# spacemeshos/go-spacemesh

Hardware: AMD Instinct MI355X
Metric: post_labels_per_sec (higher is better)
Workload: dtype u32; 1 GPU; init-mainnet-scryptN8192-4units-256GiB-sink; step_labels=2097152, scrypt_n=8192, num_units=4, labels_per_unit=4294967296, parallelism=index-range shards x1, RCCL nonce min-reduce, vrf_nonce_found=True

## Files before the change

### go-spacemesh_amd/csrc/engine.cpp

```cpp
#include "../../include/spacemesh_post.h"

#include <hip/hip_runtime.h>

#include <fcntl.h>
#include <sys/stat.h>
#include <sys/types.h>
#include <unistd.h>

#include <algorithm>
#include <array>
#include <atomic>
#include <thread>
#include <chrono>
#include <cerrno>
#include <cstdio>
#include <cstdlib>
#include <cstring>
#include <functional>
#include <map>
#include <mutex>
#include <string>
#include <vector>

#include "crypto_host.h"
#include "kernel_args.h"
#include "post_common.h"

namespace {

thread_local std::string g_last_error;

void set_error(const std::string &e) { g_last_error = e; }

int hip_fail(const char *what, hipError_t err) {
  set_error(std::string(what) + ": " + hipGetErrorString(err));
  return err == hipErrorOutOfMemory ? POST_ERR_OOM : POST_ERR;
}

#define HIP_TRY(expr)                                                          \
  do {                                                                         \
    hipError_t _e = (expr);                                                    \
    if (_e != hipSuccess) return hip_fail(#expr, _e);                          \
  } while (0)

int require_gpu(uint32_t provider_id) {
  int count = 0;
  hipError_t e = hipGetDeviceCount(&count);
  if (e != hipSuccess || count == 0) {
    set_error("no HIP device available (the HIP engine has no CPU fallback)");
    return POST_ERR_NO_GPU;
  }
  if (provider_id >= (uint32_t)count) {
    set_error("provider id out of range");
    return POST_ERR_INVALID_ARGS;
  }
  e = hipSetDevice((int)provider_id);
  if (e != hipSuccess) return hip_fail("hipSetDevice", e);
  return POST_OK;
}

void load_commitment_words(const uint8_t c[32], uint32_t w[8]) {
  std::memcpy(w, c, 32);
}

void difficulty_to_be_words(const uint8_t d[32], uint32_t w[8]) {
  for (int i = 0; i < 8; i++)
    w[i] = ((uint32_t)d[4 * i] << 24) | ((uint32_t)d[4 * i + 1] << 16) |
           ((uint32_t)d[4 * i + 2] << 8) | d[4 * i + 3];
}

constexpr uint32_t THREADS = 256;
constexpr uint32_t CAND_CAP = 1 << 16;

uint32_t pick_gap_shift(uint32_t scrypt_n) {
  const char *env = getenv("POST_GAP_SHIFT");
  if (env) {
    uint32_t g = (uint32_t)atoi(env);
    while ((scrypt_n >> g) == 0) g--;
    return g;
  }
  return 0;
}

uint64_t prove_chunk_labels() {
  const uint64_t dflt = 1ull << 24;
  const char *env = getenv("POST_PROVE_CHUNK_LABELS");
  if (!env) return dflt;
  const long long v = strtoll(env, nullptr, 10);
  if (v <= 0 || (uint64_t)v >= dflt) return dflt;
  return v < 256 ? 256 : (uint64_t)v;
}

struct VerifyWorkspace {
  std::mutex mu;
  uint32_t *d_scratch = nullptr;
  size_t scratch_cap = 0;
  uint64_t *d_idx = nullptr;
  uint32_t *d_cid = nullptr;
  uint8_t *d_out = nullptr;
  uint32_t *d_xbuf = nullptr;
  size_t tasks_cap = 0;
  uint32_t *d_cm = nullptr;
  size_t cm_cap = 0;
  uint32_t *d_vrk = nullptr;
  uint8_t *d_half = nullptr;
  uint64_t *d_vdiff = nullptr;
  size_t proofs_cap = 0;
  uint8_t *d_pass = nullptr;
};
std::mutex g_vws_mu;
std::map<int, VerifyWorkspace *> g_vws;

VerifyWorkspace *get_verify_ws(int dev) {
  std::lock_guard<std::mutex> lk(g_vws_mu);
  auto it = g_vws.find(dev);
  if (it != g_vws.end()) return it->second;
  auto *w = new VerifyWorkspace();
  g_vws[dev] = w;
  return w;
}

int ws_reserve_proofs(VerifyWorkspace *w, size_t proofs) {
  if (proofs > w->proofs_cap) {
    size_t cap = std::max<size_t>(proofs, 1024);
    if (w->d_vrk) (void)hipFree(w->d_vrk);
    if (w->d_half) (void)hipFree(w->d_half);
    if (w->d_vdiff) (void)hipFree(w->d_vdiff);
    w->d_vrk = nullptr; w->d_half = nullptr; w->d_vdiff = nullptr;
    w->proofs_cap = 0;
    HIP_TRY(hipMalloc(&w->d_vrk, cap * 44 * 4));
    HIP_TRY(hipMalloc(&w->d_half, cap));
    HIP_TRY(hipMalloc(&w->d_vdiff, cap * 8));
    w->proofs_cap = cap;
  }
  return POST_OK;
}

int ws_reserve(VerifyWorkspace *w, size_t scratch_bytes, size_t tasks,
               size_t cm_words) {
  if (scratch_bytes > w->scratch_cap) {
    if (w->d_scratch) (void)hipFree(w->d_scratch);
    w->d_scratch = nullptr;
    w->scratch_cap = 0;
    HIP_TRY(hipMalloc(&w->d_scratch, scratch_bytes));
    w->scratch_cap = scratch_bytes;
  }
  if (tasks > w->tasks_cap) {
    size_t cap = std::max<size_t>(tasks, 4096);
    if (w->d_idx) (void)hipFree(w->d_idx);
    if (w->d_cid) (void)hipFree(w->d_cid);
    if (w->d_out) (void)hipFree(w->d_out);
    if (w->d_xbuf) (void)hipFree(w->d_xbuf);
    if (w->d_pass) (void)hipFree(w->d_pass);
    w->d_idx = nullptr; w->d_cid = nullptr; w->d_out = nullptr;
    w->d_xbuf = nullptr; w->d_pass = nullptr;
    w->tasks_cap = 0;
    HIP_TRY(hipMalloc(&w->d_idx, cap * 8));
    HIP_TRY(hipMalloc(&w->d_cid, cap * 4));
    HIP_TRY(hipMalloc(&w->d_out, cap * 32));
    HIP_TRY(hipMalloc(&w->d_xbuf, cap * 128));
    HIP_TRY(hipMalloc(&w->d_pass, cap));
    w->tasks_cap = cap;
  }
  if (cm_words > w->cm_cap) {
    size_t cap = std::max<size_t>(cm_words, 1024);
    if (w->d_cm) (void)hipFree(w->d_cm);
    w->d_cm = nullptr;
    w->cm_cap = 0;
    HIP_TRY(hipMalloc(&w->d_cm, cap * 4));
    w->cm_cap = cap;
  }
  return POST_OK;
}

struct DeviceTables {
  uint32_t *d_te = nullptr;
  uint8_t *d_sbox = nullptr;
};
std::mutex g_tables_mu;
std::map<int, DeviceTables> g_tables;

int get_aes_tables(int dev, DeviceTables &out) {
  std::lock_guard<std::mutex> lk(g_tables_mu);
  auto it = g_tables.find(dev);
  if (it != g_tables.end()) {
    out = it->second;
    return POST_OK;
  }
  static uint32_t te[1024];
  static uint8_t sbox[256];
  poste::aes128_tables(te, sbox);
  DeviceTables t;
  HIP_TRY(hipMalloc(&t.d_te, sizeof(te)));
  HIP_TRY(hipMalloc(&t.d_sbox, sizeof(sbox)));
  HIP_TRY(hipMemcpy(t.d_te, te, sizeof(te), hipMemcpyHostToDevice));
  HIP_TRY(hipMemcpy(t.d_sbox, sbox, sizeof(sbox), hipMemcpyHostToDevice));
  g_tables[dev] = t;
  out = t;
  return POST_OK;
}

}

extern "C" {

const char *post_last_error(void) { return g_last_error.c_str(); }

const char *post_engine_version(void) {
  return "spacemesh-post-hip 0.2 (gfx950)";
}


int post_providers(PostProvider *providers, uint32_t cap, uint32_t *count) {
  int n = 0;
  hipError_t e = hipGetDeviceCount(&n);
  if (e != hipSuccess) n = 0;
  *count = (uint32_t)n;
  for (uint32_t i = 0; i < (uint32_t)n && i < cap; i++) {
    hipDeviceProp_t prop;
    if (hipGetDeviceProperties(&prop, (int)i) != hipSuccess) continue;
    providers[i].id = i;
    std::snprintf(providers[i].model, sizeof(providers[i].model), "%s",
                  prop.name);
    providers[i].device_type = 0;
    providers[i].memory_bytes = prop.totalGlobalMem;
    providers[i].performance = 0;
  }
  return POST_OK;
}


struct PostInitSession {
  PostInitConfig cfg;
  std::string data_dir;
  uint64_t range_start = 0, range_end = 0;
  std::atomic<uint64_t> written{0};
  std::atomic<bool> cancel{false};
  uint8_t commitment[32];

  std::mutex nonce_mu;
  bool nonce_found = false;
  uint64_t nonce_idx = 0;
  uint8_t nonce_label[32];

  uint64_t lanes = 0;
  uint64_t batch_seq = 0;
  uint32_t gap_shift = 0;
  uint64_t batch = 0;
  uint32_t *d_scratch = nullptr;
  uint8_t *d_out = nullptr;
  uint8_t *d_all = nullptr;
  bool keep_all = false;
  PostVrfCandidate *d_cand = nullptr;
  unsigned int *d_cand_count = nullptr;
  uint32_t *d_xbuf = nullptr;
  uint8_t *h_batch = nullptr;
  hipStream_t stream = nullptr;
  hipEvent_t ev0 = nullptr, ev1 = nullptr;
  double last_kernel_ms = 0;

  int split_streams = 0;
  uint32_t cand_cap = 0;
  uint8_t *d_out1 = nullptr;
  PostVrfCandidate *d_cand1 = nullptr;
  unsigned int *d_cand_count1 = nullptr;
  uint8_t *h_batch1 = nullptr;
  PostVrfCandidate *h_cand[2] = {nullptr, nullptr};
  unsigned int *h_cand_count = nullptr;
  hipStream_t stream_b = nullptr, copy_stream = nullptr;
  hipEvent_t ev_fill[4] = {nullptr, nullptr, nullptr, nullptr};
  hipEvent_t ev_tail[2][2] = {{nullptr, nullptr}, {nullptr, nullptr}};
  hipEvent_t ev_end[2] = {nullptr, nullptr}, ev_done[2] = {nullptr, nullptr};

  ~PostInitSession() {
    if (stream) (void)hipStreamSynchronize(stream);
    if (stream_b) (void)hipStreamSynchronize(stream_b);
    if (copy_stream) (void)hipStreamSynchronize(copy_stream);
    for (int i = 0; i < 4; i++)
      if (ev_fill[i]) (void)hipEventDestroy(ev_fill[i]);
    for (int i = 0; i < 2; i++) {
      for (int k = 0; k < 2; k++)
        if (ev_tail[i][k]) (void)hipEventDestroy(ev_tail[i][k]);
      if (ev_end[i]) (void)hipEventDestroy(ev_end[i]);
      if (ev_done[i]) (void)hipEventDestroy(ev_done[i]);
      if (h_cand[i]) (void)hipHostFree(h_cand[i]);
    }
    if (stream_b) (void)hipStreamDestroy(stream_b);
    if (copy_stream) (void)hipStreamDestroy(copy_stream);
    if (d_out1) (void)hipFree(d_out1);
    if (d_cand1) (void)hipFree(d_cand1);
    if (d_cand_count1) (void)hipFree(d_cand_count1);
    if (h_batch1) (void)hipHostFree(h_batch1);
    if (h_cand_count) (void)hipHostFree(h_cand_count);
    if (ev0) (void)hipEventDestroy(ev0);
    if (ev1) (void)hipEventDestroy(ev1);
    if (stream) (void)hipStreamDestroy(stream);
    if (d_scratch) (void)hipFree(d_scratch);
    if (d_out) (void)hipFree(d_out);
    if (d_all) (void)hipFree(d_all);
    if (d_cand) (void)hipFree(d_cand);
    if (d_cand_count) (void)hipFree(d_cand_count);
    if (d_xbuf) (void)hipFree(d_xbuf);
    if (h_batch) (void)hipHostFree(h_batch);
  }
};

static uint64_t existing_labels(const std::string &dir, uint64_t per_file,
                                uint64_t range_start, uint64_t range_total) {
  uint64_t done = 0;
  for (uint64_t pos = range_start; pos < range_start + range_total;) {
    uint64_t file_i = pos / per_file;
    uint64_t in_file = pos % per_file;
    uint64_t file_cap = std::min(per_file - in_file,
                                 range_start + range_total - pos);
    char path[4096];
    std::snprintf(path, sizeof path, "%s/postdata_%llu.bin", dir.c_str(),
                  (unsigned long long)file_i);
    FILE *f = std::fopen(path, "rb");
    if (!f) break;
    std::fseek(f, 0, SEEK_END);
    long sz = std::ftell(f);
    std::fclose(f);
    uint64_t labels_here = (uint64_t)(sz < 0 ? 0 : sz) / POST_LABEL_SIZE;
    if (in_file > labels_here) break;
    uint64_t usable = std::min(labels_here - in_file, file_cap);
    done += usable;
    pos += usable;
    if (usable < file_cap) break;
  }
  return done;
}

static int check_existing_metadata(PostInitSession *s);
static int write_metadata(PostInitSession *s);

int post_init_new(const PostInitConfig *cfg, PostInitSession **out) {
  if (!cfg || !out) {
    set_error("null args");
    return POST_ERR_INVALID_ARGS;
  }
  if (cfg->scrypt_n < 2 || (cfg->scrypt_n & (cfg->scrypt_n - 1))) {
    set_error("scrypt N must be a power of two >= 2");
    return POST_ERR_INVALID_ARGS;
  }
  int rc = require_gpu(cfg->provider_id);
  if (rc != POST_OK) return rc;

  struct Guard {
    PostInitSession *p;
    ~Guard() { delete p; }
  };
  auto *s = new PostInitSession();
  Guard guard{s};
  s->cfg = *cfg;
  if (cfg->data_dir) {
    s->data_dir = cfg->data_dir;
    std::string path;
    for (size_t i = 0; i <= s->data_dir.size(); i++) {
      if (i == s->data_dir.size() || s->data_dir[i] == '/') {
        path = s->data_dir.substr(0, i);
        if (!path.empty()) (void)::mkdir(path.c_str(), 0755);
      }
    }
    struct stat st;
    if (stat(s->data_dir.c_str(), &st) != 0 || !S_ISDIR(st.st_mode)) {
      set_error("cannot create data dir " + s->data_dir);
      return POST_ERR_IO;
    }
  }
  uint64_t total = (uint64_t)cfg->num_units * cfg->labels_per_unit;
  s->range_start = cfg->index_start;
  s->range_end = cfg->index_end ? cfg->index_end : total;
  if (s->range_end > total || s->range_start >= s->range_end) {
    set_error("bad index range");
    return POST_ERR_INVALID_ARGS;
  }
  poste::commitment(cfg->node_id, cfg->commitment_atx_id, s->commitment);

  s->gap_shift = pick_gap_shift(cfg->scrypt_n);
  size_t free_b = 0, total_b = 0;
  HIP_TRY(hipMemGetInfo(&free_b, &total_b));
  uint64_t budget = cfg->scratch_bytes
                        ? cfg->scratch_bytes
                        : (uint64_t)((double)free_b * 0.80);
  uint64_t per_lane = ((uint64_t)cfg->scrypt_n >> s->gap_shift) * 128;
  uint64_t lanes = budget / per_lane;
  uint64_t range = s->range_end - s->range_start;
  lanes = std::min<uint64_t>(lanes, std::max<uint64_t>(range, 64));
  lanes = std::min<uint64_t>(lanes,
                             poste_label_resident_slots(s->gap_shift));
  lanes = (lanes / 128) * 128;
  if (lanes == 0) lanes = 128;
  if (lanes == 0) {
    set_error("not enough device memory for one scratch lane block");
    return POST_ERR_OOM;
  }
  s->lanes = lanes;
  s->batch = std::min<uint64_t>(range, lanes * 4);

  HIP_TRY(hipMalloc(&s->d_scratch, (size_t)lanes * per_lane));
  uint64_t keep_bytes = range * POST_LABEL_SIZE;
  s->keep_all = s->data_dir.empty() && keep_bytes <= (8ull << 30);
  if (s->keep_all) {
    HIP_TRY(hipMalloc(&s->d_all, (size_t)keep_bytes));
  }
  HIP_TRY(hipMalloc(&s->d_out, (size_t)s->batch * POST_LABEL_SIZE));
  s->cand_cap =
      (uint32_t)std::max<uint64_t>(CAND_CAP, s->batch / 64 + 16);
  HIP_TRY(hipMalloc(&s->d_cand, sizeof(PostVrfCandidate) * s->cand_cap));
  HIP_TRY(hipMalloc(&s->d_xbuf,
                    (size_t)std::max<uint64_t>(s->batch, lanes) * 128));
  HIP_TRY(hipMalloc(&s->d_cand_count, sizeof(unsigned int)));
  HIP_TRY(hipHostMalloc(&s->h_batch, (size_t)s->batch * POST_LABEL_SIZE));
  HIP_TRY(hipStreamCreate(&s->stream));

  {
    const char *mx = getenv("POST_ROMIX_MIX");
    const bool lean = poste_label_romix_lean_ok(cfg->scrypt_n, s->gap_shift,
                                                lanes) != 0;
    if (!lean || (mx && std::strcmp(mx, "0") == 0))
      s->split_streams = 0;
    else if (mx && std::strcmp(mx, "seq") == 0)
      s->split_streams = 1;
    else
      s->split_streams = lanes >= 128 ? 2 : 0;
  }
  if (s->split_streams) {
    if (!s->keep_all)
      HIP_TRY(hipMalloc(&s->d_out1, (size_t)s->batch * POST_LABEL_SIZE));
    HIP_TRY(hipMalloc(&s->d_cand1, sizeof(PostVrfCandidate) * s->cand_cap));
    HIP_TRY(hipMalloc(&s->d_cand_count1, sizeof(unsigned int)));
    HIP_TRY(hipHostMalloc(&s->h_batch1, (size_t)s->batch * POST_LABEL_SIZE));
    HIP_TRY(hipHostMalloc(&s->h_cand_count, 2 * sizeof(unsigned int)));
    for (int i = 0; i < 2; i++) {
      HIP_TRY(hipHostMalloc(&s->h_cand[i],
                            sizeof(PostVrfCandidate) * s->cand_cap));
      HIP_TRY(hipEventCreate(&s->ev_end[i]));
      HIP_TRY(hipEventCreateWithFlags(&s->ev_done[i], hipEventDisableTiming));
      for (int k = 0; k < 2; k++)
        HIP_TRY(hipEventCreateWithFlags(&s->ev_tail[i][k],
                                        hipEventDisableTiming));
    }
    for (int i = 0; i < 4; i++)
      HIP_TRY(hipEventCreateWithFlags(&s->ev_fill[i], hipEventDisableTiming));
    if (s->split_streams == 2) HIP_TRY(hipStreamCreate(&s->stream_b));
    HIP_TRY(hipStreamCreate(&s->copy_stream));
  }

  if (!s->data_dir.empty()) {
    rc = check_existing_metadata(s);
    if (rc != POST_OK) return rc;
    rc = write_metadata(s);
    if (rc != POST_OK) return rc;
    uint64_t per_file = std::max<uint64_t>(
        1, s->cfg.max_file_size / POST_LABEL_SIZE);
    s->written = existing_labels(s->data_dir, per_file, s->range_start, range);
  }
  guard.p = nullptr;
  *out = s;
  return POST_OK;
}

uint64_t post_init_num_labels_written(const PostInitSession *s) {
  return s ? s->written.load() : 0;
}

void post_init_cancel(PostInitSession *s) {
  if (s) s->cancel = true;
}

int post_init_nonce(const PostInitSession *s, uint64_t *index,
                    uint8_t label[32]) {
  auto *m = const_cast<PostInitSession *>(s);
  std::lock_guard<std::mutex> lk(m->nonce_mu);
  if (!s->nonce_found) return POST_ERR;
  *index = s->nonce_idx;
  std::memcpy(label, s->nonce_label, 32);
  return POST_OK;
}

static int write_batch_files(PostInitSession *s, uint64_t pos, uint64_t count,
                             const uint8_t *host_labels) {
  uint64_t per_file =
      std::max<uint64_t>(1, s->cfg.max_file_size / POST_LABEL_SIZE);
  uint64_t off = 0;
  while (off < count) {
    uint64_t gpos = pos + off;
    uint64_t file_i = gpos / per_file;
    uint64_t in_file = gpos % per_file;
    uint64_t take = std::min(per_file - in_file, count - off);
    char path[4096];
    std::snprintf(path, sizeof path, "%s/postdata_%llu.bin",
                  s->data_dir.c_str(), (unsigned long long)file_i);
    FILE *f = std::fopen(path, "r+b");
    if (!f) f = std::fopen(path, "w+b");
    if (!f) {
      set_error(std::string("cannot open ") + path);
      return POST_ERR_IO;
    }
    std::fseek(f, (long)(in_file * POST_LABEL_SIZE), SEEK_SET);
    size_t wr = std::fwrite(host_labels + off * POST_LABEL_SIZE,
                            POST_LABEL_SIZE, take, f);
    std::fclose(f);
    if (wr != take) {
      set_error("short write");
      return POST_ERR_IO;
    }
    off += take;
  }
  return POST_OK;
}

static void b64(const uint8_t *in, size_t n, std::string &out) {
  static const char t[] =
      "ABCDEFGHIJKLMNOPQRSTUVWXYZabcdefghijklmnopqrstuvwxyz0123456789+/";
  for (size_t i = 0; i < n; i += 3) {
    uint32_t v = (uint32_t)in[i] << 16;
    if (i + 1 < n) v |= (uint32_t)in[i + 1] << 8;
    if (i + 2 < n) v |= in[i + 2];
    out += t[(v >> 18) & 63];
    out += t[(v >> 12) & 63];
    out += i + 1 < n ? t[(v >> 6) & 63] : '=';
    out += i + 2 < n ? t[v & 63] : '=';
  }
}

static bool b64_decode(const std::string &in, uint8_t *out, size_t want) {
  static int8_t rev[256];
  static bool init = false;
  if (!init) {
    static const char t[] =
        "ABCDEFGHIJKLMNOPQRSTUVWXYZabcdefghijklmnopqrstuvwxyz0123456789+/";
    for (int i = 0; i < 256; i++) rev[i] = -1;
    for (int i = 0; i < 64; i++) rev[(uint8_t)t[i]] = (int8_t)i;
    init = true;
  }
  size_t n = 0;
  uint32_t acc = 0;
  int bits = 0;
  for (char c : in) {
    if (c == '=') break;
    int8_t v = rev[(uint8_t)c];
    if (v < 0) return false;
    acc = (acc << 6) | (uint32_t)v;
    bits += 6;
    if (bits >= 8) {
      bits -= 8;
      if (n >= want) return false;
      out[n++] = (uint8_t)(acc >> bits);
    }
  }
  return n == want;
}

static bool md_find_string(const std::string &j, const char *key,
                           std::string &out) {
  std::string pat = std::string("\"") + key + "\": \"";
  size_t p = j.find(pat);
  if (p == std::string::npos) return false;
  p += pat.size();
  size_t e = j.find('"', p);
  if (e == std::string::npos) return false;
  out = j.substr(p, e - p);
  return true;
}

static bool md_find_u64(const std::string &j, const char *key,
                        uint64_t &out) {
  std::string pat = std::string("\"") + key + "\": ";
  size_t p = j.find(pat);
  if (p == std::string::npos) return false;
  out = strtoull(j.c_str() + p + pat.size(), nullptr, 10);
  return true;
}

static int check_existing_metadata(PostInitSession *s) {
  char path[4096];
  std::snprintf(path, sizeof path, "%s/postdata_metadata.json",
                s->data_dir.c_str());
  FILE *f = std::fopen(path, "rb");
  if (!f) return POST_OK;
  std::string j;
  char buf[4096];
  size_t rd;
  while ((rd = std::fread(buf, 1, sizeof buf, f)) > 0) j.append(buf, rd);
  std::fclose(f);
  std::string nid_b64, atx_b64, want_nid, want_atx;
  b64(s->cfg.node_id, 32, want_nid);
  b64(s->cfg.commitment_atx_id, 32, want_atx);
  uint64_t lpu = 0, n = 0;
  if (md_find_string(j, "NodeId", nid_b64) && nid_b64 != want_nid) {
    set_error("data dir belongs to a different node id (postdata_metadata"
              ".json mismatch)");
    return POST_ERR_INVALID_ARGS;
  }
  if (md_find_string(j, "CommitmentAtxId", atx_b64) &&
      atx_b64 != want_atx) {
    set_error("data dir was initialized for a different commitment ATX");
    return POST_ERR_INVALID_ARGS;
  }
  if (md_find_u64(j, "LabelsPerUnit", lpu) &&
      lpu != s->cfg.labels_per_unit) {
    set_error("data dir was initialized with a different LabelsPerUnit");
    return POST_ERR_INVALID_ARGS;
  }
  if (md_find_u64(j, "N", n) && n != s->cfg.scrypt_n) {
    set_error("data dir was initialized with different scrypt params");
    return POST_ERR_INVALID_ARGS;
  }
  uint64_t nonce_idx = 0;
  std::string nv_b64;
  if (md_find_u64(j, "Nonce", nonce_idx) &&
      md_find_string(j, "NonceValue", nv_b64)) {
    uint8_t label[32];
    if (!b64_decode(nv_b64, label, 32)) {
      set_error("postdata_metadata.json NonceValue is not 32 base64 bytes");
      return POST_ERR_INVALID_ARGS;
    }
    std::lock_guard<std::mutex> lk(s->nonce_mu);
    s->nonce_found = true;
    s->nonce_idx = nonce_idx;
    std::memcpy(s->nonce_label, label, 32);
  }
  return POST_OK;
}

static int write_metadata(PostInitSession *s) {
  std::string nid, atx, nv;
  b64(s->cfg.node_id, 32, nid);
  b64(s->cfg.commitment_atx_id, 32, atx);
  char path[4096];
  std::snprintf(path, sizeof path, "%s/postdata_metadata.json",
                s->data_dir.c_str());
  FILE *f = std::fopen(path, "w");
  if (!f) {
    set_error("cannot write metadata");
    return POST_ERR_IO;
  }
  std::fprintf(f,
               "{\n  \"NodeId\": \"%s\",\n  \"CommitmentAtxId\": \"%s\",\n"
               "  \"LabelsPerUnit\": %llu,\n  \"NumUnits\": %u,\n"
               "  \"MaxFileSize\": %llu,\n  \"Scrypt\": {\"N\": %u, \"R\": 1,"
               " \"P\": 1}",
               nid.c_str(), atx.c_str(),
               (unsigned long long)s->cfg.labels_per_unit, s->cfg.num_units,
               (unsigned long long)s->cfg.max_file_size, s->cfg.scrypt_n);
  std::lock_guard<std::mutex> lk(s->nonce_mu);
  if (s->nonce_found) {
    b64(s->nonce_label, 32, nv);
    std::fprintf(f, ",\n  \"Nonce\": %llu,\n  \"NonceValue\": \"%s\"",
                 (unsigned long long)s->nonce_idx, nv.c_str());
  }
  std::fprintf(f, "\n}\n");
  std::fclose(f);
  return POST_OK;
}

static int init_step_split(PostInitSession *s, uint64_t max_labels,
                           uint64_t *done) {
  const int ns = s->split_streams;
  const uint64_t unit = s->lanes / (uint64_t)ns;
  hipStream_t st[2] = {s->stream, s->stream_b};
  uint8_t *const d_outs[2] = {s->d_out, s->d_out1};
  uint8_t *const h_batches[2] = {s->h_batch, s->h_batch1};
  PostVrfCandidate *const d_cands[2] = {s->d_cand, s->d_cand1};
  unsigned int *const d_counts[2] = {s->d_cand_count, s->d_cand_count1};

  auto drain = [&] {
    for (int k = 0; k < ns; k++) (void)hipStreamSynchronize(st[k]);
    (void)hipStreamSynchronize(s->copy_stream);
  };
#define SPLIT_TRY(expr)                                                        \
  do {                                                                         \
    hipError_t _e = (expr);                                                    \
    if (_e != hipSuccess) {                                                    \
      drain();                                                                 \
      return hip_fail(#expr, _e);                                              \
    }                                                                          \
  } while (0)

  LabelKernelArgs args;
  std::memset(&args, 0, sizeof(args));
  load_commitment_words(s->commitment, args.commitment_le);
  args.scrypt_n = s->cfg.scrypt_n;
  args.gap_shift = s->gap_shift;
  args.scratch = s->d_scratch;
  args.scratch_lanes = s->lanes;
  args.has_difficulty = 1;
  args.cand_cap = s->cand_cap;
  RomixPhaseArgs ph;
  std::memset(&ph, 0, sizeof(ph));
  ph.scratch = s->d_scratch;
  ph.scratch_lanes = s->lanes;
  ph.slot_count = unit;
  ph.scrypt_n = s->cfg.scrypt_n;

  uint8_t cur_difficulty[32];
  std::memset(cur_difficulty, 0xff, 32);
  {
    std::lock_guard<std::mutex> lk(s->nonce_mu);
    if (s->nonce_found) std::memcpy(cur_difficulty, s->nonce_label, 32);
  }
  const char *sp_env = getenv("POST_SELFCHECK_PERIOD");
  long selfcheck_period = sp_env ? strtol(sp_env, nullptr, 10) : 1;
  if (selfcheck_period < 1) selfcheck_period = 1;

  if (!s->ev0) SPLIT_TRY(hipEventCreate(&s->ev0));
  s->last_kernel_ms = 0;

  struct Batch {
    uint64_t pos = 0, count = 0;
    uint32_t max_cand = 0;
    int set = 0;
    bool live = false;
  };
  uint64_t unit_seq = 0;
  uint64_t batch_no = 0;
  int last_set = -1;

  auto issue = [&](Batch &b) -> int {
    b.set = (int)(batch_no++ & 1);
    b.max_cand = 0;
    uint8_t *out =
        s->keep_all ? s->d_all + b.pos * POST_LABEL_SIZE : d_outs[b.set];
    args.cand = d_cands[b.set];
    args.cand_count = d_counts[b.set];
    difficulty_to_be_words(cur_difficulty, args.difficulty_be);
    SPLIT_TRY(hipMemsetAsync(d_counts[b.set], 0, sizeof(unsigned int),
                             st[unit_seq % ns]));
    bool used[2] = {false, false};
    for (uint64_t off = 0; off < b.count; off += unit) {
      const int k = (int)(unit_seq % (uint64_t)ns);
      const uint64_t c = std::min(unit, b.count - off);
      const uint32_t blocks = (uint32_t)((c + 63) / 64);
      args.start = s->range_start + b.pos + off;
      args.count = c;
      args.xbuf = s->d_xbuf + (uint64_t)k * unit * 32;
      args.out = out + off * POST_LABEL_SIZE;
      ph.xbuf = args.xbuf;
      ph.slot_base = (uint64_t)k * unit;
      ph.count = c;
      if (unit_seq == 0) SPLIT_TRY(hipEventRecord(s->ev0, st[k]));
      SPLIT_TRY(poste_launch_label_prologue(&args, blocks, st[k]));
      if (ns == 2 && unit_seq > 0)
        SPLIT_TRY(hipStreamWaitEvent(st[k], s->ev_fill[(unit_seq - 1) & 3],
                                     0));
      SPLIT_TRY(poste_launch_romix_fill(&ph, st[k]));
      if (ns == 2)
        SPLIT_TRY(hipEventRecord(s->ev_fill[unit_seq & 3], st[k]));
      SPLIT_TRY(poste_launch_romix_mix(&ph, st[k]));
      SPLIT_TRY(poste_launch_label_tail(&args, blocks, st[k]));
      b.max_cand += blocks;
      used[k] = true;
      unit_seq++;
    }
    for (int k = 0; k < ns; k++) {
      if (!used[k]) continue;
      SPLIT_TRY(hipEventRecord(s->ev_tail[b.set][k], st[k]));
      SPLIT_TRY(hipStreamWaitEvent(s->copy_stream, s->ev_tail[b.set][k], 0));
    }
    SPLIT_TRY(hipEventRecord(s->ev_end[b.set], s->copy_stream));
    SPLIT_TRY(hipMemcpyAsync(h_batches[b.set], out,
                             b.count * POST_LABEL_SIZE, hipMemcpyDeviceToHost,
                             s->copy_stream));
    SPLIT_TRY(hipMemcpyAsync(s->h_cand_count + b.set, d_counts[b.set],
                             sizeof(unsigned int), hipMemcpyDeviceToHost,
                             s->copy_stream));
    b.max_cand = std::min(b.max_cand, s->cand_cap);
    SPLIT_TRY(hipMemcpyAsync(s->h_cand[b.set], d_cands[b.set],
                             sizeof(PostVrfCandidate) * b.max_cand,
                             hipMemcpyDeviceToHost, s->copy_stream));
    SPLIT_TRY(hipEventRecord(s->ev_done[b.set], s->copy_stream));
    last_set = b.set;
    b.live = true;
    return POST_OK;
  };

  auto process = [&](Batch &b) -> int {
    b.live = false;
    const bool do_selfcheck =
        (s->batch_seq++ % (uint64_t)selfcheck_period) == 0;
    const uint64_t probe = b.count / 2;
    uint8_t ref[32];
    const int ref_rc =
        do_selfcheck
            ? poste::host_label(s->commitment, s->range_start + b.pos + probe,
                                s->cfg.scrypt_n, ref)
            : 0;
    SPLIT_TRY(hipEventSynchronize(s->ev_done[b.set]));
    const unsigned int take = std::min(s->h_cand_count[b.set], b.max_cand);
    const PostVrfCandidate *cands = s->h_cand[b.set];
    bool nonce_improved = false;
    if (take > 0) {
      std::lock_guard<std::mutex> lk(s->nonce_mu);
      for (unsigned int i = 0; i < take; i++) {
        uint8_t lab[32];
        for (int k = 0; k < 8; k++) {
          uint32_t w = cands[i].label_be[k];
          lab[4 * k] = (uint8_t)(w >> 24);
          lab[4 * k + 1] = (uint8_t)(w >> 16);
          lab[4 * k + 2] = (uint8_t)(w >> 8);
          lab[4 * k + 3] = (uint8_t)w;
        }
        int c = std::memcmp(lab, cur_difficulty, 32);
        if (!s->nonce_found || c < 0 ||
            (c == 0 && cands[i].index < s->nonce_idx)) {
          s->nonce_found = true;
          s->nonce_idx = cands[i].index;
          std::memcpy(s->nonce_label, lab, 32);
          std::memcpy(cur_difficulty, lab, 32);
          nonce_improved = true;
        }
      }
    }
    int rc = POST_OK;
    if (nonce_improved && !s->data_dir.empty()) rc = write_metadata(s);
    if (rc == POST_OK && ref_rc != 0) {
      set_error("host reference label failed");
      rc = POST_ERR;
    }
    if (rc == POST_OK && do_selfcheck &&
        std::memcmp(ref, h_batches[b.set] + probe * POST_LABEL_SIZE,
                    POST_LABEL_SIZE) != 0) {
      set_error("reference label mismatch: device labels diverge from the "
                "host reference (ErrReferenceLabelMismatch)");
      rc = POST_ERR;
    }
    if (rc == POST_OK && !s->data_dir.empty())
      rc = write_batch_files(s, s->range_start + b.pos, b.count,
                             h_batches[b.set]);
    if (rc != POST_OK) {
      drain();
      return rc;
    }
    s->written.store(b.pos + b.count);
    *done += b.count;
    return POST_OK;
  };

  const uint64_t range = s->range_end - s->range_start;
  uint64_t pos = s->written.load();
  const uint64_t target = std::min(range, pos + max_labels);
  Batch inflight[2];
  int cur = 0;
  bool cancelled = false;
  while (pos < target) {
    if (s->cancel.load()) {
      cancelled = true;
      break;
    }
    Batch &b = inflight[cur];
    b.pos = pos;
    b.count = std::min(s->batch, target - pos);
    int rc = issue(b);
    if (rc != POST_OK) return rc;
    pos += b.count;
    if (inflight[cur ^ 1].live) {
      rc = process(inflight[cur ^ 1]);
      if (rc != POST_OK) return rc;
    }
    cur ^= 1;
  }
  if (inflight[cur ^ 1].live) {
    int rc = process(inflight[cur ^ 1]);
    if (rc != POST_OK) return rc;
  }
  drain();
  if (last_set >= 0) {
    float ms = 0;
    (void)hipEventElapsedTime(&ms, s->ev0, s->ev_end[last_set]);
    s->last_kernel_ms = ms;
  }
#undef SPLIT_TRY
  return cancelled ? POST_ERR_CANCELLED : POST_OK;
}

int post_init_step(PostInitSession *s, uint64_t max_labels, uint64_t *done) {
  if (!s || !done) return POST_ERR_INVALID_ARGS;
  *done = 0;
  int rc = require_gpu(s->cfg.provider_id);
  if (rc != POST_OK) return rc;
  if (s->split_streams) return init_step_split(s, max_labels, done);

  LabelKernelArgs args;
  std::memset(&args, 0, sizeof(args));
  load_commitment_words(s->commitment, args.commitment_le);
  args.scrypt_n = s->cfg.scrypt_n;
  args.gap_shift = s->gap_shift;
  args.xbuf = s->d_xbuf;
  args.out_full = 0;
  args.scratch = s->d_scratch;
  args.scratch_lanes = s->lanes;
  args.indices = nullptr;
  args.commit_ids = nullptr;
  args.commitments = nullptr;
  args.has_difficulty = 1;
  args.cand = s->d_cand;
  args.cand_count = s->d_cand_count;
  args.cand_cap = s->cand_cap;

  uint8_t cur_difficulty[32];
  std::memset(cur_difficulty, 0xff, 32);
  {
    std::lock_guard<std::mutex> lk(s->nonce_mu);
    if (s->nonce_found) std::memcpy(cur_difficulty, s->nonce_label, 32);
  }

  const uint32_t blocks = (uint32_t)(s->lanes / 64);
  std::vector<PostVrfCandidate> cands(s->cand_cap);

  if (!s->ev0) {
    HIP_TRY(hipEventCreate(&s->ev0));
    HIP_TRY(hipEventCreate(&s->ev1));
  }
  s->last_kernel_ms = 0;

  uint64_t range = s->range_end - s->range_start;
  uint64_t pos = s->written.load();
  uint64_t target = std::min(range, pos + max_labels);
  while (pos < target) {
    if (s->cancel.load()) return POST_ERR_CANCELLED;
    uint64_t count = std::min(s->batch, target - pos);
    args.start = s->range_start + pos;
    args.count = count;
    args.out = s->keep_all ? s->d_all + pos * POST_LABEL_SIZE : s->d_out;
    difficulty_to_be_words(cur_difficulty, args.difficulty_be);
    unsigned int zero = 0;
    HIP_TRY(hipMemcpyAsync(s->d_cand_count, &zero, sizeof(zero),
                           hipMemcpyHostToDevice, s->stream));
    HIP_TRY(hipEventRecord(s->ev0, s->stream));
    HIP_TRY(poste_launch_label_kernel(&args, blocks, s->stream));
    HIP_TRY(hipEventRecord(s->ev1, s->stream));
    HIP_TRY(hipMemcpyAsync(s->h_batch, args.out, count * POST_LABEL_SIZE,
                           hipMemcpyDeviceToHost, s->stream));
    unsigned int n_cand = 0;
    HIP_TRY(hipMemcpyAsync(&n_cand, s->d_cand_count, sizeof(n_cand),
                           hipMemcpyDeviceToHost, s->stream));
    const char *sp_env = getenv("POST_SELFCHECK_PERIOD");
    long selfcheck_period = sp_env ? strtol(sp_env, nullptr, 10) : 1;
    if (selfcheck_period < 1) selfcheck_period = 1;
    const bool do_selfcheck = (s->batch_seq++ % (uint64_t)selfcheck_period)
                              == 0;
    const uint64_t probe = count / 2;
    uint8_t ref[32];
    const int ref_rc =
        do_selfcheck ? poste::host_label(s->commitment, args.start + probe,
                                         s->cfg.scrypt_n, ref)
                     : 0;
    HIP_TRY(hipStreamSynchronize(s->stream));
    bool nonce_improved = false;
    if (n_cand > 0) {
      unsigned int take = std::min(n_cand, s->cand_cap);
      HIP_TRY(hipMemcpy(cands.data(), s->d_cand,
                        sizeof(PostVrfCandidate) * take,
                        hipMemcpyDeviceToHost));
      std::lock_guard<std::mutex> lk(s->nonce_mu);
      for (unsigned int i = 0; i < take; i++) {
        uint8_t lab[32];
        for (int k = 0; k < 8; k++) {
          uint32_t w = cands[i].label_be[k];
          lab[4 * k] = (uint8_t)(w >> 24);
          lab[4 * k + 1] = (uint8_t)(w >> 16);
          lab[4 * k + 2] = (uint8_t)(w >> 8);
          lab[4 * k + 3] = (uint8_t)w;
        }
        int c = std::memcmp(lab, cur_difficulty, 32);
        if (!s->nonce_found || c < 0 ||
            (c == 0 && cands[i].index < s->nonce_idx)) {
          s->nonce_found = true;
          s->nonce_idx = cands[i].index;
          std::memcpy(s->nonce_label, lab, 32);
          std::memcpy(cur_difficulty, lab, 32);
          nonce_improved = true;
        }
      }
    }
    if (nonce_improved && !s->data_dir.empty()) {
      rc = write_metadata(s);
      if (rc != POST_OK) return rc;
    }

    if (ref_rc != 0) {
      set_error("host reference label failed");
      return POST_ERR;
    }
    if (do_selfcheck &&
        std::memcmp(ref, s->h_batch + probe * POST_LABEL_SIZE,
                    POST_LABEL_SIZE) != 0) {
      set_error("reference label mismatch: device labels diverge from the "
                "host reference (ErrReferenceLabelMismatch)");
      return POST_ERR;
    }

    if (!s->data_dir.empty()) {
      rc = write_batch_files(s, s->range_start + pos, count, s->h_batch);
      if (rc != POST_OK) return rc;
    }
    float ms = 0;
    (void)hipEventElapsedTime(&ms, s->ev0, s->ev1);
    s->last_kernel_ms += ms;
    pos += count;
    s->written.store(pos);
    *done += count;
  }
  return POST_OK;
}

double post_init_last_kernel_ms(const PostInitSession *s) {
  return s ? s->last_kernel_ms : 0.0;
}

static int nonce_only_batch(PostInitSession *s, uint64_t gstart,
                            uint64_t count) {
  LabelKernelArgs args;
  std::memset(&args, 0, sizeof(args));
  load_commitment_words(s->commitment, args.commitment_le);
  args.scrypt_n = s->cfg.scrypt_n;
  args.gap_shift = s->gap_shift;
  args.xbuf = s->d_xbuf;
  args.scratch = s->d_scratch;
  args.scratch_lanes = s->lanes;
  args.start = gstart;
  args.count = count;
  args.out = nullptr;
  args.has_difficulty = 1;
  args.cand = s->d_cand;
  args.cand_count = s->d_cand_count;
  args.cand_cap = s->cand_cap;
  uint8_t cur[32];
  std::memset(cur, 0xff, 32);
  {
    std::lock_guard<std::mutex> lk(s->nonce_mu);
    if (s->nonce_found) std::memcpy(cur, s->nonce_label, 32);
  }
  difficulty_to_be_words(cur, args.difficulty_be);
  unsigned int zero = 0;
  HIP_TRY(hipMemcpy(s->d_cand_count, &zero, sizeof(zero),
                    hipMemcpyHostToDevice));
  HIP_TRY(poste_launch_label_kernel(&args, (uint32_t)(s->lanes / 64),
                                    s->stream));
  HIP_TRY(hipStreamSynchronize(s->stream));
  unsigned int n_cand = 0;
  HIP_TRY(hipMemcpy(&n_cand, s->d_cand_count, sizeof(n_cand),
                    hipMemcpyDeviceToHost));
  if (n_cand > 0) {
    unsigned int take = std::min(n_cand, s->cand_cap);
    std::vector<PostVrfCandidate> cands(take);
    HIP_TRY(hipMemcpy(cands.data(), s->d_cand,
                      sizeof(PostVrfCandidate) * take,
                      hipMemcpyDeviceToHost));
    bool improved = false;
    {
      std::lock_guard<std::mutex> lk(s->nonce_mu);
      for (unsigned int i = 0; i < take; i++) {
        uint8_t lab[32];
        for (int k = 0; k < 8; k++) {
          uint32_t w = cands[i].label_be[k];
// ... 2094 lines not shown
```

Baseline: 2.088 million labels/s.

## Split romix work across three free-running streams by default

Adds a third compute stream and makes three-way splitting the default when there are enough lanes. Lanes now round to multiples of 64, and work units are evened out. The fill-phase event chain that serialized the two streams is now opt-in through a 'chain' mode. The stream cursor and batch parity now persist across steps, and a reset event orders the candidate-count memset before tails on other streams. The aim is more overlap between fill, mix and tail kernels, at the cost of smaller per-launch units and possible contention for memory bandwidth.

```diff
diff --git a/go-spacemesh_amd/csrc/engine.cpp b/go-spacemesh_amd/csrc/engine.cpp
--- a/go-spacemesh_amd/csrc/engine.cpp
+++ b/go-spacemesh_amd/csrc/engine.cpp
@@ -260,6 +260,9 @@
   double last_kernel_ms = 0;
 
   int split_streams = 0;
+  bool split_chain = false;
+  uint64_t unit_cursor = 0;
+  uint64_t split_batch_no = 0;
   uint32_t cand_cap = 0;
   uint8_t *d_out1 = nullptr;
   PostVrfCandidate *d_cand1 = nullptr;
@@ -267,25 +270,30 @@
   uint8_t *h_batch1 = nullptr;
   PostVrfCandidate *h_cand[2] = {nullptr, nullptr};
   unsigned int *h_cand_count = nullptr;
-  hipStream_t stream_b = nullptr, copy_stream = nullptr;
+  hipStream_t stream_b = nullptr, stream_c = nullptr, copy_stream = nullptr;
   hipEvent_t ev_fill[4] = {nullptr, nullptr, nullptr, nullptr};
-  hipEvent_t ev_tail[2][2] = {{nullptr, nullptr}, {nullptr, nullptr}};
+  hipEvent_t ev_tail[2][3] = {{nullptr, nullptr, nullptr},
+                              {nullptr, nullptr, nullptr}};
   hipEvent_t ev_end[2] = {nullptr, nullptr}, ev_done[2] = {nullptr, nullptr};
+  hipEvent_t ev_reset[2] = {nullptr, nullptr};
 
   ~PostInitSession() {
     if (stream) (void)hipStreamSynchronize(stream);
     if (stream_b) (void)hipStreamSynchronize(stream_b);
+    if (stream_c) (void)hipStreamSynchronize(stream_c);
     if (copy_stream) (void)hipStreamSynchronize(copy_stream);
     for (int i = 0; i < 4; i++)
       if (ev_fill[i]) (void)hipEventDestroy(ev_fill[i]);
     for (int i = 0; i < 2; i++) {
-      for (int k = 0; k < 2; k++)
+      for (int k = 0; k < 3; k++)
         if (ev_tail[i][k]) (void)hipEventDestroy(ev_tail[i][k]);
+      if (ev_reset[i]) (void)hipEventDestroy(ev_reset[i]);
       if (ev_end[i]) (void)hipEventDestroy(ev_end[i]);
       if (ev_done[i]) (void)hipEventDestroy(ev_done[i]);
       if (h_cand[i]) (void)hipHostFree(h_cand[i]);
     }
     if (stream_b) (void)hipStreamDestroy(stream_b);
+    if (stream_c) (void)hipStreamDestroy(stream_c);
     if (copy_stream) (void)hipStreamDestroy(copy_stream);
     if (d_out1) (void)hipFree(d_out1);
     if (d_cand1) (void)hipFree(d_cand1);
@@ -389,8 +397,11 @@
   lanes = std::min<uint64_t>(lanes, std::max<uint64_t>(range, 64));
   lanes = std::min<uint64_t>(lanes,
                              poste_label_resident_slots(s->gap_shift));
-  lanes = (lanes / 128) * 128;
-  if (lanes == 0) lanes = 128;
+  const char *const mx = getenv("POST_ROMIX_MIX");
+  const bool want3 = !mx || !*mx || std::strcmp(mx, "free3") == 0;
+  const uint64_t lane_round = want3 ? 64 : 128;
+  lanes = (lanes / lane_round) * lane_round;
+  if (lanes < 128) lanes = 128;
   if (lanes == 0) {
     set_error("not enough device memory for one scratch lane block");
     return POST_ERR_OOM;
@@ -415,15 +426,18 @@
   HIP_TRY(hipStreamCreate(&s->stream));
 
   {
-    const char *mx = getenv("POST_ROMIX_MIX");
     const bool lean = poste_label_romix_lean_ok(cfg->scrypt_n, s->gap_shift,
                                                 lanes) != 0;
     if (!lean || (mx && std::strcmp(mx, "0") == 0))
       s->split_streams = 0;
     else if (mx && std::strcmp(mx, "seq") == 0)
       s->split_streams = 1;
+    else if (want3 && lanes >= 192)
+      s->split_streams = 3;
     else
       s->split_streams = lanes >= 128 ? 2 : 0;
+    s->split_chain =
+        s->split_streams == 2 && mx && std::strcmp(mx, "chain") == 0;
   }
   if (s->split_streams) {
     if (!s->keep_all)
@@ -437,13 +451,18 @@
                             sizeof(PostVrfCandidate) * s->cand_cap));
       HIP_TRY(hipEventCreate(&s->ev_end[i]));
       HIP_TRY(hipEventCreateWithFlags(&s->ev_done[i], hipEventDisableTiming));
-      for (int k = 0; k < 2; k++)
+      HIP_TRY(hipEventCreateWithFlags(&s->ev_reset[i],
+                                      hipEventDisableTiming));
+      for (int k = 0; k < s->split_streams; k++)
         HIP_TRY(hipEventCreateWithFlags(&s->ev_tail[i][k],
                                         hipEventDisableTiming));
     }
-    for (int i = 0; i < 4; i++)
-      HIP_TRY(hipEventCreateWithFlags(&s->ev_fill[i], hipEventDisableTiming));
-    if (s->split_streams == 2) HIP_TRY(hipStreamCreate(&s->stream_b));
+    if (s->split_chain)
+      for (int i = 0; i < 4; i++)
+        HIP_TRY(hipEventCreateWithFlags(&s->ev_fill[i],
+                                        hipEventDisableTiming));
+    if (s->split_streams >= 2) HIP_TRY(hipStreamCreate(&s->stream_b));
+    if (s->split_streams >= 3) HIP_TRY(hipStreamCreate(&s->stream_c));
     HIP_TRY(hipStreamCreate(&s->copy_stream));
   }
 
@@ -659,8 +678,8 @@
 static int init_step_split(PostInitSession *s, uint64_t max_labels,
                            uint64_t *done) {
   const int ns = s->split_streams;
-  const uint64_t unit = s->lanes / (uint64_t)ns;
-  hipStream_t st[2] = {s->stream, s->stream_b};
+  const uint64_t unit = s->lanes / (uint64_t)ns / 64 * 64;
+  hipStream_t st[3] = {s->stream, s->stream_b, s->stream_c};
   uint8_t *const d_outs[2] = {s->d_out, s->d_out1};
   uint8_t *const h_batches[2] = {s->h_batch, s->h_batch1};
   PostVrfCandidate *const d_cands[2] = {s->d_cand, s->d_cand1};
@@ -714,24 +733,27 @@
     int set = 0;
     bool live = false;
   };
-  uint64_t unit_seq = 0;
-  uint64_t batch_no = 0;
+  uint64_t issued = 0;
   int last_set = -1;
 
   auto issue = [&](Batch &b) -> int {
-    b.set = (int)(batch_no++ & 1);
+    b.set = (int)(s->split_batch_no++ & 1);
     b.max_cand = 0;
     uint8_t *out =
         s->keep_all ? s->d_all + b.pos * POST_LABEL_SIZE : d_outs[b.set];
     args.cand = d_cands[b.set];
     args.cand_count = d_counts[b.set];
     difficulty_to_be_words(cur_difficulty, args.difficulty_be);
+    const int k0 = (int)(s->unit_cursor % (uint64_t)ns);
     SPLIT_TRY(hipMemsetAsync(d_counts[b.set], 0, sizeof(unsigned int),
-                             st[unit_seq % ns]));
-    bool used[2] = {false, false};
-    for (uint64_t off = 0; off < b.count; off += unit) {
-      const int k = (int)(unit_seq % (uint64_t)ns);
-      const uint64_t c = std::min(unit, b.count - off);
+                             st[k0]));
+    if (ns > 1) SPLIT_TRY(hipEventRecord(s->ev_reset[b.set], st[k0]));
+    const uint64_t nunits = (b.count + unit - 1) / unit;
+    const uint64_t per = ((b.count + nunits - 1) / nunits + 63) / 64 * 64;
+    bool used[3] = {false, false, false};
+    for (uint64_t off = 0; off < b.count; off += per) {
+      const int k = (int)(s->unit_cursor % (uint64_t)ns);
+      const uint64_t c = std::min(per, b.count - off);
       const uint32_t blocks = (uint32_t)((c + 63) / 64);
       args.start = s->range_start + b.pos + off;
       args.count = c;
@@ -740,19 +762,22 @@
       ph.xbuf = args.xbuf;
       ph.slot_base = (uint64_t)k * unit;
       ph.count = c;
-      if (unit_seq == 0) SPLIT_TRY(hipEventRecord(s->ev0, st[k]));
+      if (issued == 0) SPLIT_TRY(hipEventRecord(s->ev0, st[k]));
       SPLIT_TRY(poste_launch_label_prologue(&args, blocks, st[k]));
-      if (ns == 2 && unit_seq > 0)
-        SPLIT_TRY(hipStreamWaitEvent(st[k], s->ev_fill[(unit_seq - 1) & 3],
-                                     0));
+      if (s->split_chain && issued > 0)
+        SPLIT_TRY(hipStreamWaitEvent(
+            st[k], s->ev_fill[(s->unit_cursor - 1) & 3], 0));
       SPLIT_TRY(poste_launch_romix_fill(&ph, st[k]));
-      if (ns == 2)
-        SPLIT_TRY(hipEventRecord(s->ev_fill[unit_seq & 3], st[k]));
+      if (s->split_chain)
+        SPLIT_TRY(hipEventRecord(s->ev_fill[s->unit_cursor & 3], st[k]));
       SPLIT_TRY(poste_launch_romix_mix(&ph, st[k]));
+      if (k != k0 && !used[k])
+        SPLIT_TRY(hipStreamWaitEvent(st[k], s->ev_reset[b.set], 0));
       SPLIT_TRY(poste_launch_label_tail(&args, blocks, st[k]));
       b.max_cand += blocks;
       used[k] = true;
-      unit_seq++;
+      s->unit_cursor++;
+      issued++;
     }
     for (int k = 0; k < ns; k++) {
       if (!used[k]) continue;
```

Result: faster. 2.226 million labels/s, median of 6 (+6.6%).
